# pythoncrazy/jimm

Measured on AMD Instinct MI355X. Metric: images/sec (whole node) ViT-B/16@224 train, higher is better.
Workload: dtype bf16; 1 GPU; model=ViT-B/16@224, global_batch=1024, img_size=224, parallelism=dp1

## Files before the change

### jimm_amd/csrc/gemm.hip

```cpp

#include <torch/extension.h>
#include <ATen/hip/HIPContext.h>

#include "common.h"

namespace {

typedef short bf16x8_t __attribute__((ext_vector_type(8)));
typedef float f32x4_t __attribute__((ext_vector_type(4)));

#define MFMA16(A, B, C) __builtin_amdgcn_mfma_f32_16x16x32_bf16(A, B, C, 0, 0, 0)

constexpr int BM = 128, BN = 128, BK = 64;
constexpr int PITCH = BK + 8;



__device__ __forceinline__ void stage_tile_glds(const bf16* __restrict__ gsrc, int64_t ldg,
                                                short* lds_base, int tid) {
  const int wave = tid / WAVE;
  const int lane = tid % WAVE;
#pragma unroll
  for (int round = 0; round < 4; ++round) {
    const int off = round * 4096 + wave * 1024 + lane * 16;
    const int row = off >> 7;
    const int chunk = (off >> 4) & 7;
    const int src_chunk = chunk ^ (row & 7);
    const bf16* g = gsrc + (int64_t)row * ldg + src_chunk * 8;
    typedef const __attribute__((address_space(1))) unsigned int* gp_t;
    typedef __attribute__((address_space(3))) unsigned int* lp_t;
    __builtin_amdgcn_global_load_lds((gp_t)(const void*)g,
                                     (lp_t)(void*)(reinterpret_cast<char*>(lds_base) + round * 4096 + wave * 1024),
                                     16, 0, 0);
  }
}

__device__ __forceinline__ bf16x8_t lds_read_frag(const short* base, int row, int chunk) {
  const int byte = (row << 7) + ((chunk ^ (row & 7)) << 4);
  return *reinterpret_cast<const bf16x8_t*>(reinterpret_cast<const char*>(base) + byte);
}

template <int ACT, bool HAS_BIAS, bool HAS_RES, bool SAVE_PRE>
__global__ __launch_bounds__(256) void gemm_nt_fast_kernel(
    const bf16* __restrict__ X, const bf16* __restrict__ W, const float* __restrict__ bias,
    const bf16* __restrict__ res, bf16* __restrict__ Y, bf16* __restrict__ Z,
    int M, int N, int K) {
  extern __shared__ __attribute__((aligned(16))) char smem[];
  short* smem_s = reinterpret_cast<short*>(smem);
  auto xs = [&](int buf) { return smem_s + buf * 8192; };
  auto ws = [&](int buf) { return smem_s + 16384 + buf * 8192; };

  const int tid = threadIdx.x;
  const int lane = tid % WAVE;
  const int wave = tid / WAVE;
  const int lo = lane & 15, hi = lane >> 4;

  const int mt = M / BM, nt = N / BN;
  const int nwg = mt * nt;
  int wg = blockIdx.x;
  {
    const int q = nwg / 8, r = nwg % 8;
    const int xcd = wg % 8, idx = wg / 8;
    wg = (xcd < r ? xcd * (q + 1) : r * (q + 1) + (xcd - r) * q) + idx;
  }
  const int m0 = (wg / nt) * BM;
  const int n0 = (wg % nt) * BN;
  const int wm = (wave >> 1) * 64, wn = (wave & 1) * 64;

  f32x4_t acc[4][4] = {};

  stage_tile_glds(X + (int64_t)m0 * K, K, xs(0), tid);
  stage_tile_glds(W + (int64_t)n0 * K, K, ws(0), tid);
  __syncthreads();

  const int nk = K / BK;
  for (int kt = 0; kt < nk; ++kt) {
    const int buf = kt & 1;
    if (kt + 1 < nk) {
      stage_tile_glds(X + (int64_t)m0 * K + (kt + 1) * BK, K, xs(buf ^ 1), tid);
      stage_tile_glds(W + (int64_t)n0 * K + (kt + 1) * BK, K, ws(buf ^ 1), tid);
    }
#pragma unroll
    for (int ks = 0; ks < 2; ++ks) {
      bf16x8_t xa[4], wb[4];
#pragma unroll
      for (int mi = 0; mi < 4; ++mi) xa[mi] = lds_read_frag(xs(buf), wm + 16 * mi + lo, 4 * ks + hi);
#pragma unroll
      for (int ni = 0; ni < 4; ++ni) wb[ni] = lds_read_frag(ws(buf), wn + 16 * ni + lo, 4 * ks + hi);
#pragma unroll
      for (int mi = 0; mi < 4; ++mi)
#pragma unroll
        for (int ni = 0; ni < 4; ++ni) acc[mi][ni] = MFMA16(xa[mi], wb[ni], acc[mi][ni]);
    }
    __syncthreads();
  }

#pragma unroll
  for (int mi = 0; mi < 4; ++mi) {
#pragma unroll
    for (int r = 0; r < 4; ++r) {
      const int m = m0 + wm + 16 * mi + hi * 4 + r;
#pragma unroll
      for (int ni = 0; ni < 4; ++ni) {
        const int n = n0 + wn + 16 * ni + lo;
        float vpre = acc[mi][ni][r];
        if (HAS_BIAS) vpre += bias[n];
        if (SAVE_PRE) Z[(int64_t)m * N + n] = f2bf(vpre);
        float vy = act_fwd(vpre, ACT);
        if (HAS_RES) vy += bf2f(res[(int64_t)m * N + n]);
        Y[(int64_t)m * N + n] = f2bf(vy);
      }
    }
  }
}


template <int ACT, bool HAS_BIAS, bool HAS_RES, bool SAVE_PRE>
__global__ __launch_bounds__(256) void gemm_nt_kernel(
    const bf16* __restrict__ X, const bf16* __restrict__ W, const float* __restrict__ bias,
    const bf16* __restrict__ res, bf16* __restrict__ Y, bf16* __restrict__ Z,
    int M, int N, int K) {
  extern __shared__ __attribute__((aligned(16))) char smem[];
  short* xs = reinterpret_cast<short*>(smem);
  short* ws = xs + 2 * BM * PITCH;

  const int tid = threadIdx.x;
  const int wave = tid / WAVE;
  const int lane = tid % WAVE;
  const int lo = lane & 15, hi = lane >> 4;

  const int m0 = blockIdx.x * BM;
  const int n0 = blockIdx.y * BN;
  const int wm = (wave >> 1) * 64;
  const int wn = (wave & 1) * 64;

  f32x4_t acc[4][4] = {};

  auto stage = [&](int buf, int k0) {
    short* xd = xs + buf * BM * PITCH;
    short* wd = ws + buf * BN * PITCH;
    const int row = tid / 2;
    const int c0 = (tid & 1) * 32;
#pragma unroll
    for (int h = 0; h < 2; ++h) {
      const int cc = c0 + h * 16;
      if (m0 + row < M) {
        *reinterpret_cast<bf16x8_t*>(xd + row * PITCH + cc) =
            *reinterpret_cast<const bf16x8_t*>(X + (int64_t)(m0 + row) * K + k0 + cc);
        *reinterpret_cast<bf16x8_t*>(xd + row * PITCH + cc + 8) =
            *reinterpret_cast<const bf16x8_t*>(X + (int64_t)(m0 + row) * K + k0 + cc + 8);
      } else {
        for (int i = 0; i < 16; ++i) xd[row * PITCH + cc + i] = 0;
      }
      if (n0 + row < N) {
        *reinterpret_cast<bf16x8_t*>(wd + row * PITCH + cc) =
            *reinterpret_cast<const bf16x8_t*>(W + (int64_t)(n0 + row) * K + k0 + cc);
        *reinterpret_cast<bf16x8_t*>(wd + row * PITCH + cc + 8) =
            *reinterpret_cast<const bf16x8_t*>(W + (int64_t)(n0 + row) * K + k0 + cc + 8);
      } else {
        for (int i = 0; i < 16; ++i) wd[row * PITCH + cc + i] = 0;
      }
    }
  };

  stage(0, 0);
  __syncthreads();

  const int nk = K / BK;
  for (int kt = 0; kt < nk; ++kt) {
    const int buf = kt & 1;
    if (kt + 1 < nk) stage(buf ^ 1, (kt + 1) * BK);
    short* xd = xs + buf * BM * PITCH;
    short* wd = ws + buf * BN * PITCH;
#pragma unroll
    for (int ks = 0; ks < 2; ++ks) {
      bf16x8_t xa[4], wb[4];
#pragma unroll
      for (int mi = 0; mi < 4; ++mi)
        xa[mi] = *reinterpret_cast<const bf16x8_t*>(xd + (wm + 16 * mi + lo) * PITCH + 32 * ks + hi * 8);
#pragma unroll
      for (int ni = 0; ni < 4; ++ni)
        wb[ni] = *reinterpret_cast<const bf16x8_t*>(wd + (wn + 16 * ni + lo) * PITCH + 32 * ks + hi * 8);
#pragma unroll
      for (int mi = 0; mi < 4; ++mi)
#pragma unroll
        for (int ni = 0; ni < 4; ++ni)
          acc[mi][ni] = MFMA16(xa[mi], wb[ni], acc[mi][ni]);
    }
    __syncthreads();
  }

#pragma unroll
  for (int mi = 0; mi < 4; ++mi) {
#pragma unroll
    for (int r = 0; r < 4; ++r) {
      const int m = m0 + wm + 16 * mi + hi * 4 + r;
      if (m >= M) continue;
#pragma unroll
      for (int ni = 0; ni < 4; ++ni) {
        const int n = n0 + wn + 16 * ni + lo;
        if (n >= N) continue;
        float vpre = acc[mi][ni][r];
        if (HAS_BIAS) vpre += bias[n];
        if (SAVE_PRE) Z[(int64_t)m * N + n] = f2bf(vpre);
        float vy = act_fwd(vpre, ACT);
        if (HAS_RES) vy += bf2f(res[(int64_t)m * N + n]);
        Y[(int64_t)m * N + n] = f2bf(vy);
      }
    }
  }
}

}

bool gemm256_supported(int64_t M, int64_t N, int64_t K);
void gemm_nt_256(torch::Tensor x, torch::Tensor w, c10::optional<torch::Tensor> bias_f32,
                 std::string act, c10::optional<torch::Tensor> residual, torch::Tensor y,
                 c10::optional<torch::Tensor> z);
bool gemm8p_supported(int64_t M, int64_t N, int64_t K);
void gemm_nt_8p(torch::Tensor x, torch::Tensor w, c10::optional<torch::Tensor> bias_f32,
                std::string act, c10::optional<torch::Tensor> residual, torch::Tensor y,
                c10::optional<torch::Tensor> z);

static int gemm_tile_mode() {
  const char* env = getenv("JIMM_AMD_GEMM_TILE");
  if (!env) return 0;
  return atoi(env);
}

bool gemm_supported(int64_t M, int64_t N, int64_t K, std::string dtype) {
  if (dtype != "torch.bfloat16") return false;
  if (K % BK != 0) return false;
  const char* env = getenv("JIMM_AMD_GEMM");
  if (env && std::string(env) == "blas") return false;
  return true;
}

std::vector<torch::Tensor> linear_fwd(torch::Tensor x, torch::Tensor w,
                                      c10::optional<torch::Tensor> bias, std::string act,
                                      c10::optional<torch::Tensor> residual, bool save_z) {
  TORCH_CHECK(x.is_cuda() && x.is_contiguous() && w.is_contiguous());
  TORCH_CHECK(x.scalar_type() == torch::kBFloat16 && w.scalar_type() == torch::kBFloat16);
  const int M = x.size(0), K = x.size(1), N = w.size(0);
  TORCH_CHECK(w.size(1) == K && K % BK == 0);
  auto y = torch::empty({M, N}, x.options());
  torch::Tensor z;
  if (save_z) z = torch::empty({M, N}, x.options());
  c10::optional<torch::Tensor> bf;
  if (bias) bf = bias->contiguous().to(torch::kFloat32);
  int act_code = ACT_NONE;
  if (act == "gelu") act_code = ACT_GELU;
  else if (act == "gelu_tanh") act_code = ACT_GELU_TANH;
  else if (act == "quickgelu") act_code = ACT_QUICKGELU;
  else TORCH_CHECK(act.empty(), "unknown act ", act);

  const int tile_mode = gemm_tile_mode();
  if (tile_mode == 0 && gemm8p_supported(M, N, K)) {
    c10::optional<torch::Tensor> zopt;
    if (save_z) zopt = z;
    gemm_nt_8p(x, w, bf, act, residual, y, zopt);
    if (save_z) return {y, z};
    return {y, torch::Tensor()};
  }
  if (tile_mode != 128 && gemm256_supported(M, N, K)) {
    c10::optional<torch::Tensor> zopt;
    if (save_z) zopt = z;
    gemm_nt_256(x, w, bf, act, residual, y, zopt);
    if (save_z) return {y, z};
    return {y, torch::Tensor()};
  }

  auto stream = at::hip::getCurrentHIPStream();
  const bf16* resp = residual ? reinterpret_cast<const bf16*>(residual->data_ptr()) : nullptr;
  const float* biasp = bf ? bf->data_ptr<float>() : nullptr;
  bf16* zp = save_z ? reinterpret_cast<bf16*>(z.data_ptr()) : nullptr;
  const bool fast = (M % BM == 0) && (N % BN == 0);

#define LAUNCH(ACTC, HB, HR, SP)                                                          \
  do {                                                                                    \
    if (fast) {                                                                           \
      hipLaunchKernelGGL((gemm_nt_fast_kernel<ACTC, HB, HR, SP>),                         \
                         dim3((M / BM) * (N / BN)), dim3(256), 4 * 8192 * sizeof(short),  \
                         stream, reinterpret_cast<const bf16*>(x.data_ptr()),             \
                         reinterpret_cast<const bf16*>(w.data_ptr()), biasp, resp,        \
                         reinterpret_cast<bf16*>(y.data_ptr()), zp, M, N, K);             \
    } else {                                                                              \
      hipLaunchKernelGGL((gemm_nt_kernel<ACTC, HB, HR, SP>),                              \
                         dim3((M + BM - 1) / BM, (N + BN - 1) / BN), dim3(256),           \
                         2 * (BM + BN) * PITCH * sizeof(short), stream,                   \
                         reinterpret_cast<const bf16*>(x.data_ptr()),                     \
                         reinterpret_cast<const bf16*>(w.data_ptr()), biasp, resp,        \
                         reinterpret_cast<bf16*>(y.data_ptr()), zp, M, N, K);             \
    }                                                                                     \
  } while (0)
#define DISPATCH_ACT(HB, HR, SP)                                                          \
  switch (act_code) {                                                                     \
    case ACT_NONE: LAUNCH(ACT_NONE, HB, HR, SP); break;                                   \
    case ACT_GELU: LAUNCH(ACT_GELU, HB, HR, SP); break;                                   \
    case ACT_GELU_TANH: LAUNCH(ACT_GELU_TANH, HB, HR, SP); break;                         \
    case ACT_QUICKGELU: LAUNCH(ACT_QUICKGELU, HB, HR, SP); break;                         \
  }
  const bool hb = bias.has_value(), hr = residual.has_value();
  if (hb && hr && save_z) DISPATCH_ACT(true, true, true)
  else if (hb && hr) DISPATCH_ACT(true, true, false)
  else if (hb && save_z) DISPATCH_ACT(true, false, true)
  else if (hb) DISPATCH_ACT(true, false, false)
  else if (hr && save_z) DISPATCH_ACT(false, true, true)
  else if (hr) DISPATCH_ACT(false, true, false)
  else if (save_z) DISPATCH_ACT(false, false, true)
  else DISPATCH_ACT(false, false, false)
#undef DISPATCH_ACT
#undef LAUNCH
  if (save_z) return {y, z};
  return {y, torch::Tensor()};
}
```

### jimm_amd/csrc/gemm8p.hip

```cpp

#include <torch/extension.h>
#include <hip/hip_fp8.h>
#include <ATen/hip/HIPContext.h>

#include "common.h"

namespace {

typedef short bf16x8_t __attribute__((ext_vector_type(8)));
typedef float f32x4_t __attribute__((ext_vector_type(4)));

#define MFMA16(A, B, C) __builtin_amdgcn_mfma_f32_16x16x32_bf16(A, B, C, 0, 0, 0)

constexpr int BM = 256, BN = 256, BK = 64;
constexpr int NTHREADS = 512;
constexpr int HALF_BYTES = 128 * BK * 2;

__device__ __forceinline__ void raw_barrier() {
  asm volatile("s_barrier" ::: "memory");
}

template <bool MGUARD>
__device__ __forceinline__ const bf16* stage_base(const bf16* __restrict__ gsrc,
                                                  int64_t ldg, int row0, int rows_total,
                                                  int round, int tid) {
  const int off = round * 8192 + tid * 16;
  const int row = off >> 7;
  const int chunk = ((off >> 4) & 7) ^ (row & 7);
  int grow = row0 + row;
  if (MGUARD) grow = grow < rows_total ? grow : rows_total - 1;
  return gsrc + (int64_t)grow * ldg + chunk * 8;
}

__device__ __forceinline__ void glds16(const bf16* g, char* lds_dst) {
  typedef const __attribute__((address_space(1))) unsigned int* gp_t;
  typedef __attribute__((address_space(3))) unsigned int* lp_t;
  __builtin_amdgcn_global_load_lds((gp_t)(const void*)g, (lp_t)(void*)lds_dst, 16, 0, 0);
}

__device__ __forceinline__ bf16x8_t lds_frag8p(const char* base, int byte_off) {
  return *reinterpret_cast<const bf16x8_t*>(base + byte_off);
}

__device__ __forceinline__ int frag_off(int row, int chunk) {
  return (row << 7) + ((chunk ^ (row & 7)) << 4);
}

template <int ACT, bool HAS_BIAS, bool HAS_RES, bool SAVE_PRE, bool MGUARD, bool GRADM = false,
          bool FP8O = false>
__global__ __launch_bounds__(NTHREADS, 2) void gemm_nt_8p_kernel(
    const bf16* __restrict__ X, const bf16* __restrict__ W, const float* __restrict__ bias,
    const bf16* __restrict__ res, bf16* __restrict__ Y, bf16* __restrict__ Z,
    int M, int N, int K, unsigned char* __restrict__ Y8 = nullptr,
    const float* __restrict__ scale8 = nullptr,
    unsigned int* __restrict__ amax_bits = nullptr) {
  extern __shared__ __attribute__((aligned(16))) char smem[];
  auto As = [&](int buf, int h) { return smem + (buf * 2 + h) * HALF_BYTES; };
  auto Bs = [&](int slot, int h) {
    return smem + 4 * HALF_BYTES + (slot * 2 + h) * HALF_BYTES;
  };

  const int tid = threadIdx.x;
  const int lane = tid % WAVE;
  const int wave = tid / WAVE;
  const int lo = lane & 15, hi = lane >> 4;

  const int mt = MGUARD ? (M + BM - 1) / BM : M / BM;
  const int nt = N / BN;
  const int nwg = mt * nt;
  int wg = blockIdx.x;
  {
    const int q = nwg / 8, r = nwg % 8;
    const int xcd = wg % 8, idx = wg / 8;
    wg = (xcd < r ? xcd * (q + 1) : r * (q + 1) + (xcd - r) * q) + idx;
  }
  const int m0 = (wg / nt) * BM;
  const int n0 = (wg % nt) * BN;
  const int wm = (wave >> 2);
  const int wn = (wave & 3);

  f32x4_t acc[2][4][4] = {};

  const int nk = K / BK;
  const bf16* asrc[2][2];
  const bf16* bsrc[2][2];
#pragma unroll
  for (int h = 0; h < 2; ++h)
#pragma unroll
    for (int r = 0; r < 2; ++r) {
      asrc[h][r] = stage_base<MGUARD>(X, K, m0 + h * 128, M, r, tid);
      bsrc[h][r] = stage_base<false>(W + (int64_t)n0 * K, K, h * 128, N, r, tid);
    }
  const int ldst = tid * 16;
  auto stageA = [&](int kt, int h) {
    char* img = As(kt & 1, h);
    glds16(asrc[h][0] + (int64_t)kt * BK, img + ldst);
    glds16(asrc[h][1] + (int64_t)kt * BK, img + 8192 + ldst);
  };
  auto stageB = [&](int kt, int slot, int h) {
    char* img = Bs(slot, h);
    glds16(bsrc[h][0] + (int64_t)kt * BK, img + ldst);
    glds16(bsrc[h][1] + (int64_t)kt * BK, img + 8192 + ldst);
  };

  int offA[2][4], offB[2][4];
#pragma unroll
  for (int kh = 0; kh < 2; ++kh) {
#pragma unroll
    for (int mi = 0; mi < 4; ++mi)
      offA[kh][mi] = frag_off(wm * 64 + 16 * mi + lo, 4 * kh + hi);
#pragma unroll
    for (int ni = 0; ni < 4; ++ni)
      offB[kh][ni] = frag_off((wn & 1) * 64 + 16 * ni + lo, 4 * kh + hi);
  }
  const int bh = wn >> 1;

  stageB(0, 0, 0);
  stageB(0, 0, 1);
  stageA(0, 0);
  stageA(0, 1);
  asm volatile("s_waitcnt vmcnt(2)" ::: "memory");
  raw_barrier();

  int slot = 0, slot1 = nk > 1 ? 1 : 0;
  for (int t = 0; t < nk; ++t) {
    const int buf = t & 1;
    const char* a0i = As(buf, 0);
    const char* a1i = As(buf, 1);
    const char* bi = Bs(slot, bh);
    const bool more = t + 1 < nk;
#pragma unroll
    for (int kh = 0; kh < 2; ++kh) {
      bf16x8_t xa[4], wb[4];
#pragma unroll
      for (int mi = 0; mi < 4; ++mi) xa[mi] = lds_frag8p(a0i, offA[kh][mi]);
#pragma unroll
      for (int ni = 0; ni < 4; ++ni) wb[ni] = lds_frag8p(bi, offB[kh][ni]);
      if (more) {
        if (kh == 0) stageB(t + 1, slot1, 0);
        else stageA(t + 1, 0);
      }
      if (kh == 0) {
        if (t == nk - 1) asm volatile("s_waitcnt vmcnt(0)" ::: "memory");
        else asm volatile("s_waitcnt vmcnt(2)" ::: "memory");
      } else {
        asm volatile("s_waitcnt vmcnt(4)" ::: "memory");
      }
      raw_barrier();
      __builtin_amdgcn_s_setprio(1);
#pragma unroll
      for (int mi = 0; mi < 4; ++mi)
#pragma unroll
        for (int ni = 0; ni < 4; ++ni)
          acc[0][mi][ni] = MFMA16(xa[mi], wb[ni], acc[0][mi][ni]);
      __builtin_amdgcn_s_setprio(0);

#pragma unroll
      for (int mi = 0; mi < 4; ++mi) xa[mi] = lds_frag8p(a1i, offA[kh][mi]);
      if (more) {
        if (kh == 0) stageB(t + 1, slot1, 1);
        else stageA(t + 1, 1);
      }
      if (kh == 0) asm volatile("s_waitcnt vmcnt(4)" ::: "memory");
      else asm volatile("s_waitcnt vmcnt(2)" ::: "memory");
      raw_barrier();
      __builtin_amdgcn_s_setprio(1);
#pragma unroll
      for (int mi = 0; mi < 4; ++mi)
#pragma unroll
        for (int ni = 0; ni < 4; ++ni)
          acc[1][mi][ni] = MFMA16(xa[mi], wb[ni], acc[1][mi][ni]);
      __builtin_amdgcn_s_setprio(0);
    }
    slot = slot1;
    slot1 = slot1 + 1 == 3 ? 0 : slot1 + 1;
  }

  float rs8 = 1.f, tmax = 0.f;
  if (FP8O) rs8 = 1.f / scale8[0];
#pragma unroll
  for (int pr = 0; pr < 2; ++pr) {
#pragma unroll
    for (int mi = 0; mi < 4; ++mi) {
#pragma unroll
      for (int r = 0; r < 4; ++r) {
        const int m = m0 + pr * 128 + wm * 64 + 16 * mi + hi * 4 + r;
        if (MGUARD && m >= M) continue;
#pragma unroll
        for (int ni = 0; ni < 4; ++ni) {
          const int n = n0 + wn * 64 + 16 * ni + lo;
          float vpre = acc[pr][mi][ni][r];
          if (HAS_BIAS) vpre += bias[n];
          if (SAVE_PRE) Z[(int64_t)m * N + n] = f2bf(vpre);
          float vy;
          if (GRADM) {
            vy = vpre * act_grad(bf2f(res[(int64_t)m * N + n]), ACT);
          } else {
            vy = act_fwd(vpre, ACT);
            if (HAS_RES) vy += bf2f(res[(int64_t)m * N + n]);
          }
          Y[(int64_t)m * N + n] = f2bf(vy);
          if (FP8O) {
            tmax = fmaxf(tmax, fabsf(vy));
            Y8[(int64_t)m * N + n] = cvt_e4m3(vy * rs8);
          }
        }
      }
    }
  }
  if (FP8O) {
    tmax = wave_reduce_max(tmax);
    if (lane == 0) atomicMax(amax_bits, __float_as_uint(tmax));
  }
}

}

bool gemm8p_supported(int64_t M, int64_t N, int64_t K) {
  return M >= 1 && (N % BN == 0) && (K % BK == 0) && K >= 2 * BK;
}

torch::Tensor gemm_nt_8p_gradact(torch::Tensor dy, torch::Tensor wt, torch::Tensor z,
                                 std::string act) {
  const int M = dy.size(0), K = dy.size(1), N = wt.size(0);
  TORCH_CHECK(dy.is_contiguous() && wt.is_contiguous() && z.is_contiguous());
  TORCH_CHECK(wt.size(1) == K && z.size(0) == M && z.size(1) == N);
  TORCH_CHECK(gemm8p_supported(M, N, K));
  int act_code = ACT_NONE;
  if (act == "gelu") act_code = ACT_GELU;
  else if (act == "gelu_tanh") act_code = ACT_GELU_TANH;
  else if (act == "quickgelu") act_code = ACT_QUICKGELU;
  else TORCH_CHECK(false, "gradact needs an activation, got ", act);
  auto y = torch::empty({M, N}, dy.options());
  auto stream = at::hip::getCurrentHIPStream();
  const size_t shmem = 10 * HALF_BYTES;
  const bool mguard = (M % BM) != 0;
  const int mt = (M + BM - 1) / BM;
#define LAUNCH_GRAD(ACTC, MG)                                                              \
  do {                                                                                     \
    auto kfn = gemm_nt_8p_kernel<ACTC, false, true, false, MG, true>;                      \
    static bool attr_g_##ACTC##MG = [&] {                                                  \
      hipFuncSetAttribute(reinterpret_cast<const void*>(kfn),                              \
                          hipFuncAttributeMaxDynamicSharedMemorySize, (int)shmem);         \
      return true;                                                                         \
    }();                                                                                   \
    (void)attr_g_##ACTC##MG;                                                               \
    hipLaunchKernelGGL(kfn, dim3(mt * (N / BN)), dim3(NTHREADS), shmem, stream,            \
                       reinterpret_cast<const bf16*>(dy.data_ptr()),                       \
                       reinterpret_cast<const bf16*>(wt.data_ptr()), nullptr,              \
                       reinterpret_cast<const bf16*>(z.data_ptr()),                        \
                       reinterpret_cast<bf16*>(y.data_ptr()), nullptr, M, N, K,            \
                       nullptr, nullptr, nullptr);                                         \
  } while (0)
#define DG(ACTC)                                                                           \
  do {                                                                                     \
    if (mguard) LAUNCH_GRAD(ACTC, true);                                                   \
    else LAUNCH_GRAD(ACTC, false);                                                         \
  } while (0)
  switch (act_code) {
    case ACT_GELU: DG(ACT_GELU); break;
    case ACT_GELU_TANH: DG(ACT_GELU_TANH); break;
    case ACT_QUICKGELU: DG(ACT_QUICKGELU); break;
  }
#undef DG
#undef LAUNCH_GRAD
  return y;
}

std::vector<torch::Tensor> gemm_nt_8p_gradact_fp8(torch::Tensor dy, torch::Tensor wt,
                                                  torch::Tensor z, std::string act,
                                                  torch::Tensor scale8, torch::Tensor amax) {
  const int M = dy.size(0), K = dy.size(1), N = wt.size(0);
  TORCH_CHECK(dy.is_contiguous() && wt.is_contiguous() && z.is_contiguous());
  TORCH_CHECK(wt.size(1) == K && z.size(0) == M && z.size(1) == N);
  TORCH_CHECK(gemm8p_supported(M, N, K));
  int act_code = ACT_NONE;
  if (act == "gelu") act_code = ACT_GELU;
  else if (act == "gelu_tanh") act_code = ACT_GELU_TANH;
  else if (act == "quickgelu") act_code = ACT_QUICKGELU;
  else TORCH_CHECK(false, "gradact needs an activation, got ", act);
  auto y = torch::empty({M, N}, dy.options());
  auto y8 = torch::empty({M, N}, dy.options().dtype(torch::kUInt8));
  auto stream = at::hip::getCurrentHIPStream();
  const size_t shmem = 10 * HALF_BYTES;
  const bool mguard = (M % BM) != 0;
  const int mt = (M + BM - 1) / BM;
#define LAUNCH_GRAD8(ACTC, MG)                                                             \
  do {                                                                                     \
    auto kfn = gemm_nt_8p_kernel<ACTC, false, true, false, MG, true, true>;                \
    static bool attr_g8_##ACTC##MG = [&] {                                                 \
      hipFuncSetAttribute(reinterpret_cast<const void*>(kfn),                              \
                          hipFuncAttributeMaxDynamicSharedMemorySize, (int)shmem);         \
      return true;                                                                         \
    }();                                                                                   \
    (void)attr_g8_##ACTC##MG;                                                              \
    hipLaunchKernelGGL(kfn, dim3(mt * (N / BN)), dim3(NTHREADS), shmem, stream,            \
                       reinterpret_cast<const bf16*>(dy.data_ptr()),                       \
                       reinterpret_cast<const bf16*>(wt.data_ptr()), nullptr,              \
                       reinterpret_cast<const bf16*>(z.data_ptr()),                        \
                       reinterpret_cast<bf16*>(y.data_ptr()), nullptr, M, N, K,            \
                       y8.data_ptr<unsigned char>(), scale8.data_ptr<float>(),             \
                       reinterpret_cast<unsigned int*>(amax.data_ptr()));                  \
  } while (0)
#define DG8(ACTC)                                                                          \
  do {                                                                                     \
    if (mguard) LAUNCH_GRAD8(ACTC, true);                                                  \
    else LAUNCH_GRAD8(ACTC, false);                                                        \
  } while (0)
  switch (act_code) {
    case ACT_GELU: DG8(ACT_GELU); break;
    case ACT_GELU_TANH: DG8(ACT_GELU_TANH); break;
    case ACT_QUICKGELU: DG8(ACT_QUICKGELU); break;
  }
#undef DG8
#undef LAUNCH_GRAD8
  return {y, y8};
}

void gemm_nt_8p(torch::Tensor x, torch::Tensor w, c10::optional<torch::Tensor> bias_f32,
                std::string act, c10::optional<torch::Tensor> residual, torch::Tensor y,
                c10::optional<torch::Tensor> z) {
  const int M = x.size(0), K = x.size(1), N = w.size(0);
  TORCH_CHECK(gemm8p_supported(M, N, K));
  int act_code = ACT_NONE;
  if (act == "gelu") act_code = ACT_GELU;
  else if (act == "gelu_tanh") act_code = ACT_GELU_TANH;
  else if (act == "quickgelu") act_code = ACT_QUICKGELU;
  else TORCH_CHECK(act.empty(), "unknown act ", act);
  auto stream = at::hip::getCurrentHIPStream();
  const bf16* resp = residual ? reinterpret_cast<const bf16*>(residual->data_ptr()) : nullptr;
  const float* biasp = bias_f32 ? bias_f32->data_ptr<float>() : nullptr;
  bf16* zp = z ? reinterpret_cast<bf16*>(z->data_ptr()) : nullptr;
  const size_t shmem = 10 * HALF_BYTES;
  const bool mguard = (M % BM) != 0;
  const int mt = (M + BM - 1) / BM;

#define LAUNCH8P(ACTC, HB, HR, SP, MG)                                                     \
  do {                                                                                     \
    auto kfn = gemm_nt_8p_kernel<ACTC, HB, HR, SP, MG>;                                    \
    static bool attr_set_##ACTC##HB##HR##SP##MG = [&] {                                    \
      hipFuncSetAttribute(reinterpret_cast<const void*>(kfn),                              \
                          hipFuncAttributeMaxDynamicSharedMemorySize, (int)shmem);         \
      return true;                                                                         \
    }();                                                                                   \
    (void)attr_set_##ACTC##HB##HR##SP##MG;                                                 \
    hipLaunchKernelGGL(kfn, dim3(mt * (N / BN)), dim3(NTHREADS), shmem, stream,            \
                       reinterpret_cast<const bf16*>(x.data_ptr()),                        \
                       reinterpret_cast<const bf16*>(w.data_ptr()), biasp, resp,           \
                       reinterpret_cast<bf16*>(y.data_ptr()), zp, M, N, K,                 \
                       nullptr, nullptr, nullptr);                                         \
  } while (0)
#define DISPATCH_MG(ACTC, HB, HR, SP)                                                      \
  do {                                                                                     \
    if (mguard) LAUNCH8P(ACTC, HB, HR, SP, true);                                          \
    else LAUNCH8P(ACTC, HB, HR, SP, false);                                                \
  } while (0)
#define DISPATCH_ACT8P(HB, HR, SP)                                                         \
  switch (act_code) {                                                                      \
    case ACT_NONE: DISPATCH_MG(ACT_NONE, HB, HR, SP); break;                               \
    case ACT_GELU: DISPATCH_MG(ACT_GELU, HB, HR, SP); break;                               \
    case ACT_GELU_TANH: DISPATCH_MG(ACT_GELU_TANH, HB, HR, SP); break;                     \
    case ACT_QUICKGELU: DISPATCH_MG(ACT_QUICKGELU, HB, HR, SP); break;                     \
  }
  const bool hb = bias_f32.has_value(), hr = residual.has_value(), sp = z.has_value();
  if (hb && hr && sp) DISPATCH_ACT8P(true, true, true)
  else if (hb && hr) DISPATCH_ACT8P(true, true, false)
  else if (hb && sp) DISPATCH_ACT8P(true, false, true)
  else if (hb) DISPATCH_ACT8P(true, false, false)
  else if (hr && sp) DISPATCH_ACT8P(false, true, true)
  else if (hr) DISPATCH_ACT8P(false, true, false)
  else if (sp) DISPATCH_ACT8P(false, false, true)
  else DISPATCH_ACT8P(false, false, false)
#undef DISPATCH_ACT8P
#undef DISPATCH_MG
#undef LAUNCH8P
}
```

### jimm_amd/ops/hip_linear.py

```python

from __future__ import annotations

import os

import torch

from jimm_amd.ops import _backend



_FP8_STATE = {"enabled": False}
_FP8_MAX = 448.0


def set_fp8(on: bool = True) -> None:
    _FP8_STATE["enabled"] = bool(on)


def fp8_enabled() -> bool:
    return _FP8_STATE["enabled"]


def _fp8_ok(x2: torch.Tensor, w: torch.Tensor) -> bool:
    return (
        x2.dtype == torch.bfloat16
        and x2.shape[1] % 16 == 0
        and w.shape[0] % 16 == 0
        and hasattr(torch, "_scaled_mm")
    )


def _quant_e4m3(t: torch.Tensor):
    scale = (t.abs().amax().float() / _FP8_MAX).clamp(min=1e-12)
    t8 = (t * scale.reciprocal().to(t.dtype)).to(torch.float8_e4m3fn)
    return t8, scale


def _gemm_nt_fp8(x2: torch.Tensor, w: torch.Tensor) -> torch.Tensor:
    x8, sx = _quant_e4m3(x2)
    w8, sw = _quant_e4m3(w)
    return torch._scaled_mm(
        x8, w8.t(), scale_a=sx.view(1, 1), scale_b=sw.view(1, 1), out_dtype=torch.bfloat16
    )


def _gemm_mode() -> str:
    return os.environ.get("JIMM_AMD_GEMM", "hip")


def _deterministic() -> bool:
    return os.environ.get("JIMM_AMD_DETERMINISTIC", "0") == "1"


def _dw_ws() -> bool:
    return os.environ.get("JIMM_AMD_DW_WS", "1") != "0"


def _dw_gemm(ext, dz: torch.Tensor, x2: torch.Tensor, out_dtype) -> torch.Tensor:
    if (
        _gemm_mode() == "hip"
        and (_dw_ws() or not _deterministic())
        and dz.dtype == torch.bfloat16
        and ext.gemm_tn8p_supported(dz.shape[0], dz.shape[1], x2.shape[1])
    ):
        return ext.gemm_tn_8p(dz, x2, 0, out_dtype == torch.bfloat16).to(out_dtype)
    return torch.matmul(dz.t(), x2)


def _dw_db_gemm(ext, dz: torch.Tensor, x2: torch.Tensor, out_dtype):
    if (
        _gemm_mode() == "hip"
        and not _deterministic()
        and dz.dtype == torch.bfloat16
        and ext.gemm_tn8p_supported(dz.shape[0], dz.shape[1], x2.shape[1])
    ):
        dw, db = ext.gemm_tn_8p_db(dz, x2, 0, out_dtype == torch.bfloat16)
        return dw.to(out_dtype), db.to(dz.dtype)
    dw = torch.matmul(dz.t(), x2)
    if dz.is_cuda and dz.shape[-1] % 8 == 0:
        db = _backend.ext().colsum(dz).to(dz.dtype)
    else:
        db = dz.sum(dim=0)
    return dw, db


def _dx_gemm(ext, dz: torch.Tensor, w: torch.Tensor) -> torch.Tensor:
    if (
        _gemm_mode() == "hip"
        and dz.dtype == torch.bfloat16
        and ext.gemm8p_supported(dz.shape[0], w.shape[1], w.shape[0])
    ):
        wt = w.t().contiguous()
        y, _ = ext.linear_fwd(dz, wt, None, "", None, False)
        return y
    return torch.matmul(dz, w)


def _gemm_nt(x2: torch.Tensor, w: torch.Tensor) -> torch.Tensor:
    return torch.matmul(x2, w.t())


class _LinearActFn(torch.autograd.Function):
    @staticmethod
    def forward(ctx, x, w, b, act, residual):
        in_f, out_f = w.shape[1], w.shape[0]
        x2 = x.contiguous().reshape(-1, in_f)
        res2 = residual.contiguous().reshape(-1, out_f) if residual is not None else None
        ext = _backend.ext()
        if _FP8_STATE["enabled"] and _fp8_ok(x2, w):
            z = _gemm_nt_fp8(x2, w)
            y = ext.bias_act_fwd(z, b, act or "", res2)
        elif _gemm_mode() == "hip" and ext.gemm_supported(x2.shape[0], out_f, in_f, str(x2.dtype)):
            y, z = ext.linear_fwd(x2, w, b, act or "", res2, act is not None)
        elif act is None and res2 is None and b is not None:
            y = z = torch.addmm(b, x2, w.t())
        else:
            z = _gemm_nt(x2, w)
            y = ext.bias_act_fwd(z, b, act or "", res2)
        if act is not None:
            ctx.save_for_backward(x2, w, z)
        else:
            ctx.save_for_backward(x2, w)
        ctx.act = act
        ctx.has_bias = b is not None
        ctx.has_res = residual is not None
        ctx.res_shape = residual.shape if residual is not None else None
        ctx.x_shape = x.shape
        return y.view(*x.shape[:-1], out_f)

    @staticmethod
    def backward(ctx, dy):
        if ctx.act is not None:
            x2, w, z = ctx.saved_tensors
        else:
            x2, w = ctx.saved_tensors
            z = None
        dy2 = dy.contiguous().reshape(-1, dy.shape[-1])
        if ctx.act is not None:
            dz = _backend.ext().act_bwd(dy2, z, ctx.act)
        else:
            dz = dy2
        ext = _backend.ext()
        dx = _dx_gemm(ext, dz, w).view(ctx.x_shape) if ctx.needs_input_grad[0] else None
        if ctx.needs_input_grad[1] and ctx.has_bias and ctx.needs_input_grad[2]:
            dw, db = _dw_db_gemm(ext, dz, x2, w.dtype)
        else:
            dw = _dw_gemm(ext, dz, x2, w.dtype) if ctx.needs_input_grad[1] else None
            if ctx.has_bias and ctx.needs_input_grad[2]:
                if dz.is_cuda and dz.shape[-1] % 8 == 0:
                    db = _backend.ext().colsum(dz).to(dz.dtype)
                else:
                    db = dz.sum(dim=0)
            else:
                db = None
        dres = dy.view(ctx.res_shape) if (ctx.has_res and ctx.needs_input_grad[4]) else None
        return dx, dw, db, None, dres


def linear_act(x, w, b, act, residual):
    return _LinearActFn.apply(x, w, b, act, residual)


class _PatchEmbedFn(torch.autograd.Function):

    @staticmethod
    def forward(ctx, img, w, b, patch):
        B, C, H, W = img.shape
        h, wn = H // patch, W // patch
        ext = _backend.ext()
        cols = ext.im2col_patch(img.contiguous(), patch)
        w2 = w.reshape(w.shape[0], -1).contiguous()
        if (
            _gemm_mode() == "hip"
            and cols.dtype == torch.bfloat16
            and ext.gemm8p_supported(cols.shape[0], w2.shape[0], w2.shape[1])
        ):
            y, _ = ext.linear_fwd(cols, w2, b, "", None, False)
        else:
            z = _gemm_nt(cols, w2)
            y = ext.bias_act_fwd(z, b, "", None)
        ctx.save_for_backward(cols, w2)
        ctx.img_shape = img.shape
        ctx.patch = patch
        ctx.has_bias = b is not None
        ctx.w_shape = w.shape
        return y.view(B, h * wn, w.shape[0])

    @staticmethod
    def backward(ctx, dy):
        cols, w2 = ctx.saved_tensors
        patch = ctx.patch
        ext = _backend.ext()
        dy2 = dy.contiguous().reshape(-1, dy.shape[-1])
        dcols = _dx_gemm(ext, dy2, w2)
        dimg = ext.col2im_patch(dcols, list(ctx.img_shape), patch) if ctx.needs_input_grad[0] else None
        dw = _dw_gemm(ext, dy2, cols, w2.dtype).view(ctx.w_shape) if ctx.needs_input_grad[1] else None
        if ctx.has_bias and ctx.needs_input_grad[2]:
            if dy2.shape[-1] % 8 == 0:
                db = _backend.ext().colsum(dy2).to(dy2.dtype)
            else:
                db = dy2.sum(dim=0)
        else:
            db = None
        return dimg, dw, db, None


def patch_embed(img, w, b, patch):
    return _PatchEmbedFn.apply(img, w, b, patch)
```

Measured before the change: 5976 images/sec.

## Vectorize 8p GEMM epilogue via transposed MFMA and permuted W rows; skip unused patch dx

Swaps the MFMA operand order and permutes the rows of W as they are staged, so each lane's accumulators cover 16 consecutive output columns. The epilogue can then use 16-byte vector loads and stores for bias, residual, Y, Z and the FP8 output instead of scalar strided accesses. Bias is passed in its native bf16/fp32 dtype, which avoids a per-call conversion to fp32. The patch-embed backward also skips the dx GEMM and col2im when the image needs no gradient. The risk is mapping bugs in the permutation, which static_asserts partly guard.

```diff
diff --git a/jimm_amd/csrc/gemm.hip b/jimm_amd/csrc/gemm.hip
--- a/jimm_amd/csrc/gemm.hip
+++ b/jimm_amd/csrc/gemm.hip
@@ -218,7 +218,7 @@
                  std::string act, c10::optional<torch::Tensor> residual, torch::Tensor y,
                  c10::optional<torch::Tensor> z);
 bool gemm8p_supported(int64_t M, int64_t N, int64_t K);
-void gemm_nt_8p(torch::Tensor x, torch::Tensor w, c10::optional<torch::Tensor> bias_f32,
+void gemm_nt_8p(torch::Tensor x, torch::Tensor w, c10::optional<torch::Tensor> bias,
                 std::string act, c10::optional<torch::Tensor> residual, torch::Tensor y,
                 c10::optional<torch::Tensor> z);
 
@@ -246,8 +246,6 @@
   auto y = torch::empty({M, N}, x.options());
   torch::Tensor z;
   if (save_z) z = torch::empty({M, N}, x.options());
-  c10::optional<torch::Tensor> bf;
-  if (bias) bf = bias->contiguous().to(torch::kFloat32);
   int act_code = ACT_NONE;
   if (act == "gelu") act_code = ACT_GELU;
   else if (act == "gelu_tanh") act_code = ACT_GELU_TANH;
@@ -258,10 +256,18 @@
   if (tile_mode == 0 && gemm8p_supported(M, N, K)) {
     c10::optional<torch::Tensor> zopt;
     if (save_z) zopt = z;
-    gemm_nt_8p(x, w, bf, act, residual, y, zopt);
+    c10::optional<torch::Tensor> b8;
+    if (bias) {
+      const bool native = bias->scalar_type() == torch::kBFloat16 ||
+                          bias->scalar_type() == torch::kFloat32;
+      b8 = native ? bias->contiguous() : bias->contiguous().to(torch::kFloat32);
+    }
+    gemm_nt_8p(x, w, b8, act, residual, y, zopt);
     if (save_z) return {y, z};
     return {y, torch::Tensor()};
   }
+  c10::optional<torch::Tensor> bf;
+  if (bias) bf = bias->contiguous().to(torch::kFloat32);
   if (tile_mode != 128 && gemm256_supported(M, N, K)) {
     c10::optional<torch::Tensor> zopt;
     if (save_z) zopt = z;
diff --git a/jimm_amd/csrc/gemm8p.hip b/jimm_amd/csrc/gemm8p.hip
--- a/jimm_amd/csrc/gemm8p.hip
+++ b/jimm_amd/csrc/gemm8p.hip
@@ -16,18 +16,46 @@
 constexpr int NTHREADS = 512;
 constexpr int HALF_BYTES = 128 * BK * 2;
 
+constexpr int sigma_row(int rho) {
+  return (((rho & 15) >> 2) << 4) + ((rho >> 4) << 2) + (rho & 3);
+}
+constexpr int epi_col(int hi, int ni, int r) { return sigma_row(16 * ni + 4 * hi + r); }
+
+constexpr bool sigma_is_involutive_bijection() {
+  unsigned long long seen = 0;
+  for (int rho = 0; rho < 64; ++rho) {
+    const int s = sigma_row(rho);
+    if (s < 0 || s >= 64 || sigma_row(s) != rho) return false;
+    seen |= 1ull << s;
+  }
+  return seen == ~0ull;
+}
+constexpr bool lane_cols_are_contiguous() {
+  for (int hi = 0; hi < 4; ++hi) {
+    if ((epi_col(hi, 0, 0) * 2) % 16 != 0) return false;
+    if (epi_col(hi, 0, 0) != 16 * hi) return false;
+    for (int ni = 0; ni < 4; ++ni)
+      for (int r = 0; r < 4; ++r)
+        if (epi_col(hi, ni, r) != epi_col(hi, 0, 0) + 4 * ni + r) return false;
+  }
+  return true;
+}
+static_assert(sigma_is_involutive_bijection(), "sigma_row must permute 0..63 (and be its own inverse)");
+static_assert(lane_cols_are_contiguous(),
+              "a lane's 16 accumulator columns must be consecutive and 16-byte aligned");
+
 __device__ __forceinline__ void raw_barrier() {
   asm volatile("s_barrier" ::: "memory");
 }
 
-template <bool MGUARD>
+template <bool MGUARD, bool PERM = false>
 __device__ __forceinline__ const bf16* stage_base(const bf16* __restrict__ gsrc,
                                                   int64_t ldg, int row0, int rows_total,
                                                   int round, int tid) {
   const int off = round * 8192 + tid * 16;
   const int row = off >> 7;
   const int chunk = ((off >> 4) & 7) ^ (row & 7);
-  int grow = row0 + row;
+  int grow = row0 + (PERM ? (row & ~63) + sigma_row(row & 63) : row);
   if (MGUARD) grow = grow < rows_total ? grow : rows_total - 1;
   return gsrc + (int64_t)grow * ldg + chunk * 8;
 }
@@ -46,14 +74,24 @@
   return (row << 7) + ((chunk ^ (row & 7)) << 4);
 }
 
+__device__ __forceinline__ unsigned int cvt4_e4m3(float a, float b, float c, float d) {
+  a = fminf(fmaxf(a, -448.f), 448.f);
+  b = fminf(fmaxf(b, -448.f), 448.f);
+  c = fminf(fmaxf(c, -448.f), 448.f);
+  d = fminf(fmaxf(d, -448.f), 448.f);
+  int v = __builtin_amdgcn_cvt_pk_fp8_f32(a, b, 0, false);
+  v = __builtin_amdgcn_cvt_pk_fp8_f32(c, d, v, true);
+  return (unsigned int)v;
+}
+
 template <int ACT, bool HAS_BIAS, bool HAS_RES, bool SAVE_PRE, bool MGUARD, bool GRADM = false,
           bool FP8O = false>
 __global__ __launch_bounds__(NTHREADS, 2) void gemm_nt_8p_kernel(
-    const bf16* __restrict__ X, const bf16* __restrict__ W, const float* __restrict__ bias,
+    const bf16* __restrict__ X, const bf16* __restrict__ W, const void* __restrict__ bias,
     const bf16* __restrict__ res, bf16* __restrict__ Y, bf16* __restrict__ Z,
     int M, int N, int K, unsigned char* __restrict__ Y8 = nullptr,
     const float* __restrict__ scale8 = nullptr,
-    unsigned int* __restrict__ amax_bits = nullptr) {
+    unsigned int* __restrict__ amax_bits = nullptr, int bias_bf16 = 0) {
   extern __shared__ __attribute__((aligned(16))) char smem[];
   auto As = [&](int buf, int h) { return smem + (buf * 2 + h) * HALF_BYTES; };
   auto Bs = [&](int slot, int h) {
@@ -89,7 +127,7 @@
 #pragma unroll
     for (int r = 0; r < 2; ++r) {
       asrc[h][r] = stage_base<MGUARD>(X, K, m0 + h * 128, M, r, tid);
-      bsrc[h][r] = stage_base<false>(W + (int64_t)n0 * K, K, h * 128, N, r, tid);
+      bsrc[h][r] = stage_base<false, true>(W + (int64_t)n0 * K, K, h * 128, N, r, tid);
     }
   const int ldst = tid * 16;
   auto stageA = [&](int kt, int h) {
@@ -152,7 +190,7 @@
       for (int mi = 0; mi < 4; ++mi)
 #pragma unroll
         for (int ni = 0; ni < 4; ++ni)
-          acc[0][mi][ni] = MFMA16(xa[mi], wb[ni], acc[0][mi][ni]);
+          acc[0][mi][ni] = MFMA16(wb[ni], xa[mi], acc[0][mi][ni]);
       __builtin_amdgcn_s_setprio(0);
 
 #pragma unroll
@@ -169,7 +207,7 @@
       for (int mi = 0; mi < 4; ++mi)
 #pragma unroll
         for (int ni = 0; ni < 4; ++ni)
-          acc[1][mi][ni] = MFMA16(xa[mi], wb[ni], acc[1][mi][ni]);
+          acc[1][mi][ni] = MFMA16(wb[ni], xa[mi], acc[1][mi][ni]);
       __builtin_amdgcn_s_setprio(0);
     }
     slot = slot1;
@@ -178,33 +216,55 @@
 
   float rs8 = 1.f, tmax = 0.f;
   if (FP8O) rs8 = 1.f / scale8[0];
+  const int nb = n0 + wn * 64 + epi_col(hi, 0, 0);
+  float bv[16];
+  if (HAS_BIAS) {
+    if (bias_bf16) vload_f32<16>(reinterpret_cast<const bf16*>(bias) + nb, bv);
+    else vload_f32<16>(reinterpret_cast<const float*>(bias) + nb, bv);
+  }
 #pragma unroll
   for (int pr = 0; pr < 2; ++pr) {
 #pragma unroll
     for (int mi = 0; mi < 4; ++mi) {
-#pragma unroll
-      for (int r = 0; r < 4; ++r) {
-        const int m = m0 + pr * 128 + wm * 64 + 16 * mi + hi * 4 + r;
-        if (MGUARD && m >= M) continue;
-#pragma unroll
-        for (int ni = 0; ni < 4; ++ni) {
-          const int n = n0 + wn * 64 + 16 * ni + lo;
-          float vpre = acc[pr][mi][ni][r];
-          if (HAS_BIAS) vpre += bias[n];
-          if (SAVE_PRE) Z[(int64_t)m * N + n] = f2bf(vpre);
-          float vy;
+      const int m = m0 + pr * 128 + wm * 64 + 16 * mi + lo;
+      if (MGUARD && m >= M) continue;
+      const int64_t o = (int64_t)m * N + nb;
+      bf16x8_t rv[2];
+      if (HAS_RES) {
+        rv[0] = *reinterpret_cast<const bf16x8_t*>(res + o);
+        rv[1] = *reinterpret_cast<const bf16x8_t*>(res + o + 8);
+      }
+      unsigned int q8[4];
+#pragma unroll
+      for (int h = 0; h < 2; ++h) {
+        bf16x8_t zv, yv;
+        float vy[8];
+#pragma unroll
+        for (int j = 0; j < 8; ++j) {
+          const int c = 8 * h + j;
+          float vpre = acc[pr][mi][c >> 2][c & 3];
+          if (HAS_BIAS) vpre += bv[c];
+          if (SAVE_PRE) zv[j] = f2bfs(vpre);
           if (GRADM) {
-            vy = vpre * act_grad(bf2f(res[(int64_t)m * N + n]), ACT);
+            vy[j] = vpre * act_grad(bfs2f(rv[h][j]), ACT);
           } else {
-            vy = act_fwd(vpre, ACT);
-            if (HAS_RES) vy += bf2f(res[(int64_t)m * N + n]);
+            vy[j] = act_fwd(vpre, ACT);
+            if (HAS_RES) vy[j] += bfs2f(rv[h][j]);
           }
-          Y[(int64_t)m * N + n] = f2bf(vy);
-          if (FP8O) {
-            tmax = fmaxf(tmax, fabsf(vy));
-            Y8[(int64_t)m * N + n] = cvt_e4m3(vy * rs8);
-          }
+          yv[j] = f2bfs(vy[j]);
+          if (FP8O) tmax = fmaxf(tmax, fabsf(vy[j]));
         }
+        if (SAVE_PRE) *reinterpret_cast<bf16x8_t*>(Z + o + 8 * h) = zv;
+        *reinterpret_cast<bf16x8_t*>(Y + o + 8 * h) = yv;
+        if (FP8O) {
+          q8[2 * h] = cvt4_e4m3(vy[0] * rs8, vy[1] * rs8, vy[2] * rs8, vy[3] * rs8);
+          q8[2 * h + 1] = cvt4_e4m3(vy[4] * rs8, vy[5] * rs8, vy[6] * rs8, vy[7] * rs8);
+        }
+      }
+      if (FP8O) {
+        typedef unsigned int u32x4_t __attribute__((ext_vector_type(4)));
+        u32x4_t q = {q8[0], q8[1], q8[2], q8[3]};
+        *reinterpret_cast<u32x4_t*>(Y8 + o) = q;
       }
     }
   }
@@ -250,7 +310,7 @@
                        reinterpret_cast<const bf16*>(wt.data_ptr()), nullptr,              \
                        reinterpret_cast<const bf16*>(z.data_ptr()),                        \
                        reinterpret_cast<bf16*>(y.data_ptr()), nullptr, M, N, K,            \
-                       nullptr, nullptr, nullptr);                                         \
+                       nullptr, nullptr, nullptr, 0);                                      \
   } while (0)
 #define DG(ACTC)                                                                           \
   do {                                                                                     \
@@ -300,7 +360,7 @@
                        reinterpret_cast<const bf16*>(z.data_ptr()),                        \
                        reinterpret_cast<bf16*>(y.data_ptr()), nullptr, M, N, K,            \
                        y8.data_ptr<unsigned char>(), scale8.data_ptr<float>(),             \
-                       reinterpret_cast<unsigned int*>(amax.data_ptr()));                  \
+                       reinterpret_cast<unsigned int*>(amax.data_ptr()), 0);               \
   } while (0)
 #define DG8(ACTC)                                                                          \
   do {                                                                                     \
@@ -317,11 +377,15 @@
   return {y, y8};
 }
 
-void gemm_nt_8p(torch::Tensor x, torch::Tensor w, c10::optional<torch::Tensor> bias_f32,
+void gemm_nt_8p(torch::Tensor x, torch::Tensor w, c10::optional<torch::Tensor> bias,
                 std::string act, c10::optional<torch::Tensor> residual, torch::Tensor y,
                 c10::optional<torch::Tensor> z) {
   const int M = x.size(0), K = x.size(1), N = w.size(0);
   TORCH_CHECK(gemm8p_supported(M, N, K));
+  TORCH_CHECK(!bias || (bias->is_contiguous() && bias->numel() == N &&
+                        (bias->scalar_type() == torch::kBFloat16 ||
+                         bias->scalar_type() == torch::kFloat32)),
+              "gemm_nt_8p: bias must be contiguous bf16 or fp32 of N elements");
   int act_code = ACT_NONE;
   if (act == "gelu") act_code = ACT_GELU;
   else if (act == "gelu_tanh") act_code = ACT_GELU_TANH;
@@ -329,7 +393,8 @@
   else TORCH_CHECK(act.empty(), "unknown act ", act);
   auto stream = at::hip::getCurrentHIPStream();
   const bf16* resp = residual ? reinterpret_cast<const bf16*>(residual->data_ptr()) : nullptr;
-  const float* biasp = bias_f32 ? bias_f32->data_ptr<float>() : nullptr;
+  const void* biasp = bias ? bias->data_ptr() : nullptr;
+  const int bias_bf16 = bias && bias->scalar_type() == torch::kBFloat16;
   bf16* zp = z ? reinterpret_cast<bf16*>(z->data_ptr()) : nullptr;
   const size_t shmem = 10 * HALF_BYTES;
   const bool mguard = (M % BM) != 0;
@@ -348,7 +413,7 @@
                        reinterpret_cast<const bf16*>(x.data_ptr()),                        \
                        reinterpret_cast<const bf16*>(w.data_ptr()), biasp, resp,           \
                        reinterpret_cast<bf16*>(y.data_ptr()), zp, M, N, K,                 \
-                       nullptr, nullptr, nullptr);                                         \
+                       nullptr, nullptr, nullptr, bias_bf16);                              \
   } while (0)
 #define DISPATCH_MG(ACTC, HB, HR, SP)                                                      \
   do {                                                                                     \
@@ -362,7 +427,7 @@
     case ACT_GELU_TANH: DISPATCH_MG(ACT_GELU_TANH, HB, HR, SP); break;                     \
     case ACT_QUICKGELU: DISPATCH_MG(ACT_QUICKGELU, HB, HR, SP); break;                     \
   }
-  const bool hb = bias_f32.has_value(), hr = residual.has_value(), sp = z.has_value();
+  const bool hb = bias.has_value(), hr = residual.has_value(), sp = z.has_value();
   if (hb && hr && sp) DISPATCH_ACT8P(true, true, true)
   else if (hb && hr) DISPATCH_ACT8P(true, true, false)
   else if (hb && sp) DISPATCH_ACT8P(true, false, true)
diff --git a/jimm_amd/ops/hip_linear.py b/jimm_amd/ops/hip_linear.py
--- a/jimm_amd/ops/hip_linear.py
+++ b/jimm_amd/ops/hip_linear.py
@@ -192,8 +192,10 @@
         patch = ctx.patch
         ext = _backend.ext()
         dy2 = dy.contiguous().reshape(-1, dy.shape[-1])
-        dcols = _dx_gemm(ext, dy2, w2)
-        dimg = ext.col2im_patch(dcols, list(ctx.img_shape), patch) if ctx.needs_input_grad[0] else None
+        dimg = None
+        if ctx.needs_input_grad[0]:
+            dcols = _dx_gemm(ext, dy2, w2)
+            dimg = ext.col2im_patch(dcols, list(ctx.img_shape), patch)
         dw = _dw_gemm(ext, dy2, cols, w2.dtype).view(ctx.w_shape) if ctx.needs_input_grad[1] else None
         if ctx.has_bias and ctx.needs_input_grad[2]:
             if dy2.shape[-1] % 8 == 0:
```

New measurement: 6051 images/sec, median of 5. 1.01x the previous value.
